# hidayetersindursun/LangSplatV2

Measured on AMD Instinct MI355X. Metric: frames/s fwd+bwd @ 1M Gaussians 1080p 3+16ch; achieved HBM GB/s, higher is better.
Workload: dtype f32; 1 GPU; BASELINE cfg3: 1M Gaussians, 1920x1080, SH deg 3 + 16 dense language channels, fwd+bwd, all inputs require grad; 1 view per GPU; gaussians=1000000, width=1920, height=1080, lang_dim=16, sh_degree=3, global_batch=1, parallelism=single GPU

## Files before the change

### langsplatv2_amd/csrc/binning.hip

```cpp
#include "bin_common.h"

#include <algorithm>

#ifndef LSR_BIN_TARGET
#define LSR_BIN_TARGET 512
#endif
#ifndef LSR_SORT_WAVE_MAX
#define LSR_SORT_WAVE_MAX 1024
#endif
#ifndef LSR_SORT_DPP
#define LSR_SORT_DPP 1
#endif

namespace lsr {

#define SCAN_ITEMS 16
#define SCAN_BLOCK 256
#define SCAN_TILE (SCAN_ITEMS * SCAN_BLOCK)

size_t scan_partials(size_t n) { return (n + SCAN_TILE - 1) / SCAN_TILE + 1; }

template <int NB>
__device__ __forceinline__ uint64_t block_excl_scan_u64_n(uint64_t v, uint64_t* sh, uint64_t& total)
{
    const int lane = threadIdx.x & 63, w = threadIdx.x >> 6;
    uint64_t x = v;
#pragma unroll
    for (int d = 1; d < 64; d <<= 1) {
        uint64_t y = __shfl_up(x, d, 64);
        if (lane >= d) x += y;
    }
    if (lane == 63) sh[w] = x;
    __syncthreads();
    uint64_t wofs = 0, tot = 0;
    for (int k = 0; k < NB / 64; k++) {
        if (k < w) wofs += sh[k];
        tot += sh[k];
    }
    __syncthreads();
    total = tot;
    return wofs + x - v;
}
__device__ __forceinline__ uint64_t block_excl_scan_u64(uint64_t v, uint64_t* sh, uint64_t& total)
{
    return block_excl_scan_u64_n<SCAN_BLOCK>(v, sh, total);
}

__global__ void __launch_bounds__(SCAN_BLOCK) k_scan_reduce(const uint32_t* __restrict__ in, size_t n,
                                                            uint64_t* __restrict__ part)
{
    __shared__ uint64_t sh[SCAN_BLOCK / 64];
    const size_t base = (size_t)blockIdx.x * SCAN_TILE + (size_t)threadIdx.x * SCAN_ITEMS;
    uint64_t s = 0;
#pragma unroll
    for (int k = 0; k < SCAN_ITEMS; k++)
        if (base + k < n) s += in[base + k];
    uint64_t tot;
    block_excl_scan_u64(s, sh, tot);
    if (threadIdx.x == 0) part[blockIdx.x] = tot;
}

__global__ void __launch_bounds__(SCAN_BLOCK) k_scan_part(uint64_t* __restrict__ part, int nb)
{
    __shared__ uint64_t sh[SCAN_BLOCK / 64];
    uint64_t carry = 0;
    for (int base = 0; base < nb; base += SCAN_BLOCK) {
        const int i = base + threadIdx.x;
        uint64_t v = i < nb ? part[i] : 0;
        uint64_t tot;
        uint64_t ex = block_excl_scan_u64(v, sh, tot);
        __syncthreads();
        if (i < nb) part[i] = carry + ex;
        carry += tot;
        __syncthreads();
    }
    if (threadIdx.x == 0) part[nb] = carry;
}

__global__ void __launch_bounds__(SCAN_BLOCK) k_scan_apply(const uint32_t* __restrict__ in, uint32_t* __restrict__ out,
                                                           size_t n, const uint64_t* __restrict__ part, int exclusive)
{
    __shared__ uint64_t sh[SCAN_BLOCK / 64];
    const size_t base = (size_t)blockIdx.x * SCAN_TILE + (size_t)threadIdx.x * SCAN_ITEMS;
    uint32_t v[SCAN_ITEMS];
    uint64_t s = 0;
#pragma unroll
    for (int k = 0; k < SCAN_ITEMS; k++) {
        v[k] = (base + k < n) ? in[base + k] : 0u;
        s += v[k];
    }
    uint64_t tot;
    uint64_t run = block_excl_scan_u64(s, sh, tot) + part[blockIdx.x];
#pragma unroll
    for (int k = 0; k < SCAN_ITEMS; k++) {
        const uint64_t incl = run + v[k];
        if (base + k < n) out[base + k] = (uint32_t)(exclusive ? run : incl);
        run = incl;
    }
}

hipError_t launch_scan_u32(const uint32_t* in, uint32_t* out, uint64_t* part, size_t n, bool exclusive, hipStream_t st)
{
    const int nb = (int)((n + SCAN_TILE - 1) / SCAN_TILE);
    if (nb > 0) k_scan_reduce<<<nb, SCAN_BLOCK, 0, st>>>(in, n, part);
    k_scan_part<<<1, SCAN_BLOCK, 0, st>>>(part, nb);
    if (nb > 0) k_scan_apply<<<nb, SCAN_BLOCK, 0, st>>>(in, out, n, part, exclusive ? 1 : 0);
    return hipGetLastError();
}

__global__ void k_publish_total(const uint64_t* __restrict__ total, uint32_t* __restrict__ tile_end,
                                uint64_t* host_slot, uint32_t seq, const uint32_t* __restrict__ cls_cnt)
{
    const uint64_t m = *total;
    const uint32_t m32 = m >= 0xffffffffull ? 0xffffffffu : (uint32_t)m;
    if (tile_end) *tile_end = m32;
    if (cls_cnt) {
        uint32_t* h = (uint32_t*)(host_slot + 1);
#pragma unroll
        for (int k = 0; k < SORT_NCLS; k++) h[k] = cls_cnt[k];
        __atomic_store_n(host_slot + LSR_CLS_SLOT, ((uint64_t)seq << 32) | m32, __ATOMIC_RELEASE);
    }
    __atomic_store_n(host_slot, ((uint64_t)seq << 32) | m32, __ATOMIC_RELEASE);
}

hipError_t launch_publish_total(const uint64_t* total, uint32_t* tile_end, uint64_t* host_slot, uint32_t seq,
                                const uint32_t* cls_cnt, hipStream_t st)
{
    k_publish_total<<<1, 1, 0, st>>>(total, tile_end, host_slot, seq, cls_cnt);
    return hipGetLastError();
}

__device__ __forceinline__ int tile_class(int n)
{
    if (n <= 0) return -1;
    if (n <= LSR_SORT_WAVE_MAX) return 0;
    if (n <= 1024) return 1;
    if (n <= 2048) return 2;
    if (n <= 4096) return 3;
    if (n <= 8192) return 4;
    return 5;
}

__device__ __forceinline__ void tile_class_append(bool active, int t, int n, int T, uint32_t* __restrict__ cls_cnt,
                                                  uint32_t* __restrict__ cls_list)
{
    const int c = active ? tile_class(n) : -1;
    const int lane = threadIdx.x & 63;
    const uint64_t below = lane ? (~0ull >> (64 - lane)) : 0ull;
    uint64_t m[SORT_NCLS];
    uint32_t cnt = 0;
#pragma unroll
    for (int k = 0; k < SORT_NCLS; k++) {
        m[k] = __ballot(c == k);
        cnt = lane == k ? (uint32_t)__popcll(m[k]) : cnt;
    }
    uint32_t base = 0;
    if (cnt) base = atomicAdd(&cls_cnt[lane], cnt);
    uint64_t mine = 0;
#pragma unroll
    for (int k = 0; k < SORT_NCLS; k++) mine = c == k ? m[k] : mine;
    const uint32_t b = __shfl(base, c < 0 ? 0 : c, 64);
    if (c >= 0) cls_list[(size_t)c * T + b + __popcll(mine & below)] = (uint32_t)t;
}

__global__ void __launch_bounds__(256) k_tile_classify(int T, const uint32_t* __restrict__ tile_start,
                                                       uint32_t* __restrict__ cls_cnt, uint32_t* __restrict__ cls_list)
{
    const int t = blockIdx.x * 256 + threadIdx.x;
    const int n = t < T ? (int)(tile_start[t + 1] - tile_start[t]) : 0;
    tile_class_append(t < T, t, n, T, cls_cnt, cls_list);
}

__global__ void __launch_bounds__(256) k_duplicate(Cam c, int P, const uint8_t* __restrict__ geom,
                                                   const int32_t* __restrict__ radii, uint32_t* __restrict__ tile_cnt,
                                                   uint32_t* __restrict__ rank)
{
    const int i = blockIdx.x * blockDim.x + threadIdx.x;
    if (i >= P) return;
    const int r = radii[i];
    if (r <= 0) return;
    const GeomLayout L = geom_layout(P);
    const float4 A = ((const float4*)(geom + L.splatA))[i];
    const float4 B = ((const float4*)(geom + L.splatB))[i];
    const uint32_t* tiles = (const uint32_t*)(geom + L.tiles);
    const uint32_t* offs = (const uint32_t*)(geom + L.offsets);
    uint32_t o = offs[i] - tiles[i];
    int x0, y0, x1, y1;
    get_rect(A.x, A.y, r, c.gx, c.gy, x0, y0, x1, y1);
    const SpanPrep sp = span_prep(A, B);
    int bx0 = x0, by0 = y0, bx1 = x1, by1 = y1;
    cull_box(A.x, A.y, A.z, A.w, B.x, B.z, bx0, by0, bx1, by1);
    for (int y = y0; y < y1; y++) {
        int sx0 = 0, sx1 = 0;
        if (y >= by0 && y < by1) row_span(sp, y, bx0, bx1, sx0, sx1);
        for (int x = x0; x < x1; x++, o++)
            rank[o] = (x >= sx0 && x < sx1) ? atomicAdd(&tile_cnt[y * c.gx + x], 1u) : 0xffffffffu;
    }
}

hipError_t launch_duplicate(const Cam& c, int P, const uint8_t* geom, const int32_t* radii, uint32_t* tile_cnt,
                            uint32_t* rank, hipStream_t st)
{
    if (P == 0) return hipSuccess;
    k_duplicate<<<(P + 255) / 256, 256, 0, st>>>(c, P, geom, radii, tile_cnt, rank);
    return hipGetLastError();
}

__global__ void __launch_bounds__(256) k_scatter(Cam c, int P, const uint8_t* __restrict__ geom,
                                                 const int32_t* __restrict__ radii,
                                                 const uint32_t* __restrict__ tile_start,
                                                 const uint32_t* __restrict__ rank, uint64_t* __restrict__ keys)
{
    const int i = blockIdx.x * blockDim.x + threadIdx.x;
    if (i >= P) return;
    const int r = radii[i];
    if (r <= 0) return;
    const GeomLayout L = geom_layout(P);
    const float4 A = ((const float4*)(geom + L.splatA))[i];
    const float depth = ((const float*)(geom + L.depth))[i];
    const uint32_t* tiles = (const uint32_t*)(geom + L.tiles);
    const uint32_t* offs = (const uint32_t*)(geom + L.offsets);
    uint32_t o = offs[i] - tiles[i];
    const uint64_t key = ((uint64_t)__float_as_uint(depth) << 32) | (uint32_t)i;
    int x0, y0, x1, y1;
    get_rect(A.x, A.y, r, c.gx, c.gy, x0, y0, x1, y1);
    for (int y = y0; y < y1; y++)
        for (int x = x0; x < x1; x++, o++)
            if (rank[o] != 0xffffffffu) keys[tile_start[y * c.gx + x] + rank[o]] = key;
}

hipError_t launch_scatter(const Cam& c, int P, const uint8_t* geom, const int32_t* radii, const uint32_t* tile_start,
                          const uint32_t* rank, uint64_t* keys, hipStream_t st)
{
    if (P == 0) return hipSuccess;
    k_scatter<<<(P + 255) / 256, 256, 0, st>>>(c, P, geom, radii, tile_start, rank, keys);
    return hipGetLastError();
}



struct WaveSpans {
    int rpre[65];
    int epre[65];
    float4 P0[64];
    float4 P1[64];
    float me[64];
    int box[64];
    int y0[64];
    int ent[64];
};

__device__ __forceinline__ int wave_spans_stage(WaveSpans& ws, int h, int bx0, int bx1, int y0, const SpanPrep& sp)
{
    const int lane = threadIdx.x & 63;
    ws.P0[lane] = make_float4(sp.x, sp.y, sp.vm, sp.vr);
    ws.P1[lane] = make_float4(sp.cb, sp.det, sp.tca, sp.ica);
    ws.me[lane] = sp.me;
    ws.box[lane] = bx0 | (bx1 << 16);
    ws.y0[lane] = y0;
    int s = h;
#pragma unroll
    for (int d = 1; d < 64; d <<= 1) {
        const int t = __shfl_up(s, d, 64);
        if (lane >= d) s += t;
    }
    ws.rpre[lane] = s - h;
    if (lane == 63) ws.rpre[64] = s;
    wave_lds_fence();
    return __shfl(s, 63, 64);
}

__device__ __forceinline__ int row_entry(const WaveSpans& ws, int e, int ty0, int& sx0, int& sx1, int& yr)
{
    const int o = wave_search(ws.rpre, e);
    yr = ws.y0[o] + (e - ws.rpre[o]);
    const float4 p0 = ws.P0[o], p1 = ws.P1[o];
    const SpanPrep sp{p0.x, p0.y, p0.z, p0.w, p1.x, p1.y, p1.z, p1.w, ws.me[o]};
    const int bx = ws.box[o];
    row_span(sp, yr + ty0, bx & 0xffff, bx >> 16, sx0, sx1);
    return o;
}

__device__ __forceinline__ int wave_spans_round(WaveSpans& ws, int r0, int R, int ty0)
{
    const int lane = threadIdx.x & 63;
    const int e = r0 + lane;
    int wd = 0, packed = 0;
    if (e < R) {
        int sx0, sx1, yr;
        const int o = row_entry(ws, e, ty0, sx0, sx1, yr);
        wd = sx1 - sx0;
        packed = sx0 | (yr << 16) | (o << 24);
    }
    int s = wd;
#pragma unroll
    for (int d = 1; d < 64; d <<= 1) {
        const int t = __shfl_up(s, d, 64);
        if (lane >= d) s += t;
    }
    ws.epre[lane] = s - wd;
    if (lane == 63) ws.epre[64] = s;
    ws.ent[lane] = packed;
    wave_lds_fence();
    return __shfl(s, 63, 64);
}

struct SpanWalk {
    int j, x, xe, y, o;
    __device__ __forceinline__ void enter(const WaveSpans& ws, int k0)
    {
        const int p = ws.ent[j];
        x = (p & 0xffff) + k0;
        xe = (p & 0xffff) + (ws.epre[j + 1] - ws.epre[j]);
        y = (p >> 16) & 0xff;
        o = p >> 24;
    }
    __device__ __forceinline__ SpanWalk(const WaveSpans& ws, int k)
    {
        j = wave_search(ws.epre, k);
        enter(ws, k - ws.epre[j]);
    }
    __device__ __forceinline__ void next(const WaveSpans& ws)
    {
        if (++x < xe) return;
        do { ++j; } while (ws.epre[j + 1] == ws.epre[j]);
        enter(ws, 0);
    }
};

__device__ __forceinline__ int stage_gaussian(WaveSpans& ws, const Cam& c, const Band& bd, const BinRec& g)
{
    int x0, x1, y0;
    const int h = band_box(c, bd, g, x0, x1, y0);
    return wave_spans_stage(ws, h, x0, x1, y0, span_prep(g.A, g.B));
}

template <int BB>
__global__ void __launch_bounds__(BB) k_bin_count(Cam c, int P, int chunk, int rows, int S,
                                                         const uint8_t* __restrict__ geom,
                                                         const int32_t* __restrict__ radii, uint32_t* __restrict__ table,
                                                         uint32_t* __restrict__ cls_cnt, uint64_t* host_slot, uint32_t seq)
{
    extern __shared__ uint32_t hist[];
    __shared__ WaveSpans wss[BB / 64];
    __shared__ uint64_t s_tot;
    const int T = c.gx * c.gy;
#if LSR_COUNT_XCD
    const int o = xcd_remap(blockIdx.x, gridDim.x);
    const int blk = o / S;
    const Band bd(c, rows, o - blk * S);
#else
    const int blk = blockIdx.x;
    const Band bd(c, rows, blockIdx.y);
#endif
    if (blockIdx.x == 0 && blockIdx.y == 0 && threadIdx.x < SORT_NCLS) cls_cnt[threadIdx.x] = 0;
    if (blockIdx.x == 0 && blockIdx.y == 0 && threadIdx.x == 0) cls_cnt[LSR_TICKET_WORD] = 0;
    for (int k = threadIdx.x; k < bd.nt; k += BB) hist[k] = 0;
    if (threadIdx.x == 0) s_tot = 0;
    __syncthreads();
    WaveSpans& ws = wss[threadIdx.x >> 6];
    const int lane = threadIdx.x & 63;
    const int g0 = blk * chunk, g1 = min(P, g0 + chunk);
    BinRec nx;
    if (g0 < g1) nx.load(geom, P, g1, radii, g0 + (threadIdx.x & ~63) + lane, false);
    for (int i0 = g0 + (threadIdx.x & ~63); i0 < g1; i0 += BB) {
        const BinRec cur = nx;
        nx.load(geom, P, g1, radii, i0 + BB + lane, false);
        const int R = stage_gaussian(ws, c, bd, cur);
        for (int e = lane; e < R; e += 64) {
            int sx0, sx1, yr;
            row_entry(ws, e, bd.ty0, sx0, sx1, yr);
            if (sx1 > sx0) {
                atomicAdd(&hist[yr * c.gx + sx0], 1u);
                if (sx1 < c.gx) atomicAdd(&hist[yr * c.gx + sx1], 0xffffffffu);
            }
        }
        wave_lds_fence();
    }
    __syncthreads();
    uint32_t* row = table + (size_t)blk * table_stride(T) + bd.t0;
    const int nrows = bd.ty1 - bd.ty0;
    uint64_t mine = 0;
    for (int r = threadIdx.x >> 6; r < nrows; r += BB / 64) {
        uint32_t carry = 0;
        for (int x0 = 0; x0 < c.gx; x0 += 64) {
            const int x = x0 + lane;
            uint32_t v = x < c.gx ? hist[r * c.gx + x] : 0u;
#pragma unroll
            for (int d = 1; d < 64; d <<= 1) {
                const uint32_t t = __shfl_up(v, d, 64);
                if (lane >= d) v += t;
            }
            if (x < c.gx) {
                row[r * c.gx + x] = carry + v;
                mine += carry + v;
            }
            carry += __shfl(v, 63, 64);
        }
    }
#pragma unroll
    for (int d = 32; d >= 1; d >>= 1) mine += __shfl_xor(mine, d, 64);
    if (lane == 0 && mine) atomicAdd((unsigned long long*)&s_tot, (unsigned long long)mine);
    __syncthreads();
    if (threadIdx.x == 0) {
        const uint64_t add = s_tot + (1ull << 44);
        const uint64_t prev = __hip_atomic_fetch_add((uint64_t*)(cls_cnt + LSR_COUNT_WORD), add, __ATOMIC_RELAXED,
                                                     __HIP_MEMORY_SCOPE_AGENT);
        if ((prev >> 44) == (uint64_t)gridDim.x * gridDim.y - 1) {
            const uint64_t m = (prev + add) & ((1ull << 44) - 1);
            const uint32_t m32 = m >= 0xffffffffull ? 0xffffffffu : (uint32_t)m;
            __hip_atomic_store(host_slot, ((uint64_t)seq << 32) | m32, __ATOMIC_RELAXED, __HIP_MEMORY_SCOPE_SYSTEM);
        }
    }
}

#define TBL_TILES 64
#define TBL_RPT 16
struct BinPublish {
    uint64_t* gpart;
    uint32_t* ticket;
    uint32_t* tile_end;
    uint64_t* host_slot;
    uint32_t seq;
};
__device__ __forceinline__ uint32_t u4_get(const uint4& v, int j) { return j == 0 ? v.x : j == 1 ? v.y : j == 2 ? v.z : v.w; }
__device__ __forceinline__ uint4 u4_add(const uint4& a, const uint4& b)
{
    return make_uint4(a.x + b.x, a.y + b.y, a.z + b.z, a.w + b.w);
}

template <int SEGS>
__global__ void __launch_bounds__(16 * SEGS) k_bin_table(int T, int Tp, int B, uint32_t* __restrict__ table,
                                                         uint32_t* __restrict__ tile_cnt,
                                                         uint32_t* __restrict__ cls_cnt,
                                                         uint32_t* __restrict__ cls_list, BinPublish pb)
{
    constexpr int NT = 16 * SEGS;
    __shared__ uint4 seg_sum[SEGS][16];
    __shared__ uint64_t sh[NT / 64];
    __shared__ int s_last;
    const int cg = threadIdx.x & 15, seg = threadIdx.x >> 4;
    const int t4 = blockIdx.x * TBL_TILES + cg * 4;
    const int b0 = seg * TBL_RPT;
    const uint4 cmask = make_uint4(t4 < T ? ~0u : 0u, t4 + 1 < T ? ~0u : 0u, t4 + 2 < T ? ~0u : 0u,
                                   t4 + 3 < T ? ~0u : 0u);
    const bool colok = t4 < Tp;
    uint4 v[TBL_RPT];
    uint4 sum = make_uint4(0u, 0u, 0u, 0u);
#pragma unroll
    for (int k = 0; k < TBL_RPT; k++) {
        const int b = b0 + k;
        uint4 x = make_uint4(0u, 0u, 0u, 0u);
        if (colok && b < B) x = *reinterpret_cast<const uint4*>(table + (size_t)b * Tp + t4);
        v[k] = make_uint4(x.x & cmask.x, x.y & cmask.y, x.z & cmask.z, x.w & cmask.w);
        sum = u4_add(sum, v[k]);
    }
    seg_sum[seg][cg] = sum;
    __syncthreads();
    uint4 run = make_uint4(0u, 0u, 0u, 0u), tot = run;
    for (int k = 0; k < SEGS; k++) {
        const uint4 x = seg_sum[k][cg];
        if (k < seg) run = u4_add(run, x);
        tot = u4_add(tot, x);
    }
    if (threadIdx.x < 64) {
        const int l = threadIdx.x, src = l >> 2, j = l & 3;
        const uint32_t n0 = __shfl(tot.x, src, 64), n1 = __shfl(tot.y, src, 64);
        const uint32_t n2 = __shfl(tot.z, src, 64), n3 = __shfl(tot.w, src, 64);
        const uint32_t nl = j == 0 ? n0 : j == 1 ? n1 : j == 2 ? n2 : n3;
        const int tl = blockIdx.x * TBL_TILES + l;
        tile_class_append(tl < T, tl, (int)nl, T, cls_cnt, cls_list);
        uint64_t g = seg == 0 ? (uint64_t)tot.x + tot.y + tot.z + tot.w : 0ull;
#pragma unroll
        for (int d = 8; d >= 1; d >>= 1) g += __shfl_xor(g, d, 64);
        if (threadIdx.x == 0) __hip_atomic_store(&pb.gpart[blockIdx.x], g, __ATOMIC_RELAXED, __HIP_MEMORY_SCOPE_AGENT);
        if (seg == 0) {
#pragma unroll
            for (int j = 0; j < 4; j++)
                if (t4 + j < T) tile_cnt[t4 + j] = u4_get(tot, j);
        }
    }
    if (colok) {
#pragma unroll
        for (int k = 0; k < TBL_RPT; k++) {
            const int b = b0 + k;
            if (b < B) *reinterpret_cast<uint4*>(table + (size_t)b * Tp + t4) = run;
            run = u4_add(run, v[k]);
        }
    }
    asm volatile("s_waitcnt vmcnt(0)" ::: "memory");
    __syncthreads();
    if (threadIdx.x == 0) {
        const uint32_t prev = __hip_atomic_fetch_add(pb.ticket, 1u, __ATOMIC_RELAXED, __HIP_MEMORY_SCOPE_AGENT);
        s_last = prev == gridDim.x - 1;
    }
    __syncthreads();
    if (!s_last) return;
    __builtin_amdgcn_fence(__ATOMIC_ACQUIRE, "wavefront");
    const int G = (int)gridDim.x;
    uint64_t carry = 0;
    for (int base = 0; base < G; base += NT * 8) {
        const int i0 = base + threadIdx.x * 8;
        uint64_t gv[8], s = 0;
#pragma unroll
        for (int k = 0; k < 8; k++)
            gv[k] = i0 + k < G ? __hip_atomic_load(&pb.gpart[i0 + k], __ATOMIC_RELAXED, __HIP_MEMORY_SCOPE_AGENT) : 0ull;
#pragma unroll
        for (int k = 0; k < 8; k++) s += gv[k];
        uint64_t gt;
        uint64_t r = carry + block_excl_scan_u64_n<NT>(s, sh, gt);
#pragma unroll
        for (int k = 0; k < 8; k++) {
            if (i0 + k < G) pb.gpart[i0 + k] = r;
            r += gv[k];
        }
        carry += gt;
    }
    if (threadIdx.x < 64) {
        const int l = threadIdx.x;
        const uint32_t cnt = l < SORT_NCLS ? __hip_atomic_load(&cls_cnt[l], __ATOMIC_RELAXED, __HIP_MEMORY_SCOPE_AGENT) : 0u;
        uint32_t cv[SORT_NCLS];
#pragma unroll
        for (int k = 0; k < SORT_NCLS; k++) cv[k] = __shfl(cnt, k, 64);
        if (l == 0) {
            const uint32_t m32 = carry >= 0xffffffffull ? 0xffffffffu : (uint32_t)carry;
            pb.gpart[G] = carry;
            *pb.tile_end = m32;
            uint32_t* h = (uint32_t*)(pb.host_slot - LSR_CLS_SLOT + 1);
#pragma unroll
            for (int k = 0; k < SORT_NCLS; k++) __hip_atomic_store(&h[k], cv[k], __ATOMIC_RELAXED, __HIP_MEMORY_SCOPE_SYSTEM);
            asm volatile("s_waitcnt vmcnt(0)" ::: "memory");
            __hip_atomic_store(pb.host_slot, ((uint64_t)pb.seq << 32) | m32, __ATOMIC_RELAXED, __HIP_MEMORY_SCOPE_SYSTEM);
        }
    }
}

__global__ void __launch_bounds__(256) k_tile_start_apply(int T, const uint32_t* __restrict__ tile_cnt,
                                                          const uint64_t* __restrict__ gpart,
                                                          uint32_t* __restrict__ tile_start)
{
    const int t = blockIdx.x * 256 + threadIdx.x;
    const uint32_t v = t < T ? tile_cnt[t] : 0u;
    uint32_t x = v;
    const int l = threadIdx.x & 63;
#pragma unroll
    for (int d = 1; d < 64; d <<= 1) {
        const uint32_t y = __shfl_up(x, d, 64);
        if (l >= d) x += y;
    }
    if (t < T) tile_start[t] = (uint32_t)gpart[t / TBL_TILES] + x - v;
}

template <int BB>
__global__ void __launch_bounds__(BB) k_bin_scatter(Cam c, int P, int chunk, int km, int rows, int S,
                                                           const uint8_t* __restrict__ geom,
                                                           const int32_t* __restrict__ radii,
                                                           const uint32_t* __restrict__ table,
                                                           const uint32_t* __restrict__ tile_start,
                                                           uint64_t* __restrict__ keys)
{
    extern __shared__ uint32_t base[];
    __shared__ WaveSpans wss[BB / 64];
    __shared__ uint64_t wkey[BB];
    const int T = c.gx * c.gy;
    const int o = xcd_remap(blockIdx.x, gridDim.x);
    const int blk = (o / S) * km;
    const Band bd(c, rows, o - (o / S) * S);
    const uint32_t* row = table + (size_t)blk * table_stride(T) + bd.t0;
    for (int k = threadIdx.x; k < bd.nt; k += BB) base[k] = tile_start[bd.t0 + k] + row[k];
    __syncthreads();
    WaveSpans& ws = wss[threadIdx.x >> 6];
    uint64_t* const key = wkey + (threadIdx.x & ~63);
    const int lane = threadIdx.x & 63;
    const int g0 = blk * chunk, g1 = min(P, g0 + km * chunk);
    BinRec nx;
    if (g0 < g1) nx.load(geom, P, g1, radii, g0 + (threadIdx.x & ~63) + lane, true);
    for (int i0 = g0 + (threadIdx.x & ~63); i0 < g1; i0 += BB) {
        const int i = i0 + lane;
        const BinRec cur = nx;
        nx.load(geom, P, g1, radii, i0 + BB + lane, true);
        key[lane] = ((uint64_t)__float_as_uint(cur.depth) << 32) | (uint32_t)i;
        const int R = stage_gaussian(ws, c, bd, cur);
        for (int r0 = 0; r0 < R; r0 += 64) {
            const int K = wave_spans_round(ws, r0, R, bd.ty0);
            const int q = (K + 63) >> 6;
            int k = lane * q;
            const int kend = min(K, k + q);
            if (k < kend) {
                SpanWalk sw(ws, k);
                for (;;) {
                    const uint32_t sa = atomicAdd(&base[sw.y * c.gx + sw.x], 1u);
                    const uint64_t ka = key[sw.o];
                    const bool two = k + 1 < kend;
                    uint32_t sb = 0;
                    uint64_t kb = 0;
                    if (two) {
                        sw.next(ws);
                        sb = atomicAdd(&base[sw.y * c.gx + sw.x], 1u);
                        kb = key[sw.o];
                    }
                    keys[sa] = ka;
                    if (two) keys[sb] = kb;
                    k += 2;
                    if (k >= kend) break;
                    sw.next(ws);
                }
            }
            wave_lds_fence();
        }
    }
}

#ifndef LSR_BAND_ROWS
#define LSR_BAND_ROWS 34
#endif
#ifndef LSR_BAND_ROWS_SMALL
#define LSR_BAND_ROWS_SMALL 68
#endif
static int bin_band_rows(const Cam& c, int P)
{
    const bool big = P >= (4 << 20);
    const int cap = big ? LSR_BAND_ROWS : LSR_BAND_ROWS_SMALL;
    const int lds = big ? LSR_BAND_LDS : 2 * LSR_BAND_LDS;
    return std::max(1, std::min(std::min(c.gy, cap), lds / (4 * c.gx)));
}

#ifndef LSR_SCATTER_LDS
#define LSR_SCATTER_LDS LSR_BAND_LDS
#endif
#ifndef LSR_SCATTER_ROWS
#define LSR_SCATTER_ROWS 0
#endif
#ifndef LSR_SCATTER_MERGE
#define LSR_SCATTER_MERGE 0
#endif
int scatter_merge(int P) { return LSR_SCATTER_MERGE > 0 ? LSR_SCATTER_MERGE : (P >= (4 << 20) ? 4 : 1); }
int bin_scatter_rows(const Cam& c)
{
    if (LSR_SCATTER_ROWS > 0) return std::max(1, std::min(c.gy, LSR_SCATTER_ROWS));
    return std::max(1, std::min(c.gy, LSR_SCATTER_LDS / (4 * c.gx)));
}

int bin_block(int P) { return P >= (4 << 20) ? 512 : 1024; }

int bin_blocks(int P, const Cam& c, int& chunk)
{
    const int rows = bin_band_rows(c, P);
    const int S = (c.gy + rows - 1) / rows;
    const int total = P >= (4 << 20) ? 2 * LSR_BIN_TARGET : LSR_BIN_TARGET;
    const int target = std::max(64, total / S);
    chunk = max(1024, (P + target - 1) / target);
    const int bb = bin_block(P);
    chunk = (chunk + bb - 1) / bb * bb;
    return (P + chunk - 1) / chunk;
}

bool bin_privatised_ok(const Cam& c) { return (size_t)c.gx * 4 <= LSR_BAND_LDS && (size_t)c.gx * c.gy <= (1u << 20); }

hipError_t launch_bin_count(const Cam& c, int P, int chunk, int B, const uint8_t* geom, const int32_t* radii,
                            uint32_t* table, uint32_t* tile_cnt, uint32_t* tile_start, uint64_t* tpart,
                            uint32_t* cls_cnt, uint32_t* cls_list, uint64_t* host_slot, uint32_t seq, hipStream_t st)
{
    const int T = c.gx * c.gy;
    const int rows = bin_band_rows(c, P);
    const int S = (c.gy + rows - 1) / rows;
    const dim3 grid(LSR_COUNT_XCD ? B * S : B, LSR_COUNT_XCD ? 1 : S);
    const size_t lds = (size_t)rows * c.gx * 4;
    if (lds > 65536) {
        (void)hipFuncSetAttribute((const void*)k_bin_count<512>, hipFuncAttributeMaxDynamicSharedMemorySize, (int)lds);
        (void)hipFuncSetAttribute((const void*)k_bin_scatter<512>, hipFuncAttributeMaxDynamicSharedMemorySize, (int)lds);
        (void)hipFuncSetAttribute((const void*)k_bin_scatter<1024>, hipFuncAttributeMaxDynamicSharedMemorySize, (int)lds);
    }
    if (B > 0) {
        if ((size_t)grid.x * grid.y >= (1u << 20)) return hipErrorInvalidValue;
        k_bin_count<512><<<grid, 512, lds, st>>>(c, P, chunk, rows, S, geom, radii, table, cls_cnt, host_slot, seq);
        BinPublish pb{tpart, cls_cnt + LSR_TICKET_WORD, tile_start + T, host_slot + LSR_CLS_SLOT, seq};
        const int G = (T + TBL_TILES - 1) / TBL_TILES, Tp = table_stride(T);
        if (B <= 16 * TBL_RPT)
            k_bin_table<16><<<G, 256, 0, st>>>(T, Tp, B, table, tile_cnt, cls_cnt, cls_list, pb);
        else if (B <= 32 * TBL_RPT)
            k_bin_table<32><<<G, 512, 0, st>>>(T, Tp, B, table, tile_cnt, cls_cnt, cls_list, pb);
        else if (B <= 64 * TBL_RPT)
            k_bin_table<64><<<G, 1024, 0, st>>>(T, Tp, B, table, tile_cnt, cls_cnt, cls_list, pb);
        else
            return hipErrorInvalidValue;
    } else {
        (void)hipMemsetAsync(tile_cnt, 0, (size_t)T * 4, st);
        (void)hipMemsetAsync(cls_cnt, 0, SORT_NCLS * 4, st);
        (void)launch_scan_u32(tile_cnt, tile_start, tpart, (size_t)T, true, st);
        (void)launch_publish_total(tpart + (scan_partials((size_t)T) - 1), tile_start + T, host_slot, seq, cls_cnt, st);
    }
    return hipGetLastError();
}

hipError_t launch_tile_start_apply(int T, int B, const uint32_t* tile_cnt, const uint64_t* tpart, uint32_t* tile_start,
                                   hipStream_t st)
{
    if (B > 0 && T > 0) k_tile_start_apply<<<(T + 255) / 256, 256, 0, st>>>(T, tile_cnt, tpart, tile_start);
    return hipGetLastError();
}

hipError_t launch_bin_scatter(const Cam& c, int P, int chunk, int B, const uint8_t* geom, const int32_t* radii,
                              const uint32_t* table, const uint32_t* tile_start, uint64_t* keys, hipStream_t st)
{
    const int rows = bin_scatter_rows(c);
    const int S = (c.gy + rows - 1) / rows;
    const size_t lds = (size_t)rows * c.gx * 4;
    if (lds > 65536) {
        (void)hipFuncSetAttribute((const void*)k_bin_scatter<512>, hipFuncAttributeMaxDynamicSharedMemorySize, (int)lds);
        (void)hipFuncSetAttribute((const void*)k_bin_scatter<1024>, hipFuncAttributeMaxDynamicSharedMemorySize, (int)lds);
    }
    const int km = scatter_merge(P), Bs = (B + km - 1) / km;
    if (B > 0 && bin_block(P) == 1024)
        k_bin_scatter<1024><<<Bs * S, 1024, lds, st>>>(c, P, chunk, km, rows, S, geom, radii, table, tile_start, keys);
    else if (B > 0)
        k_bin_scatter<512><<<Bs * S, 512, lds, st>>>(c, P, chunk, km, rows, S, geom, radii, table, tile_start, keys);
    return hipGetLastError();
}

#define SORT_BLOCK 256
#define SORT_CHUNK 4096

__device__ __forceinline__ void ce(uint64_t* a, int i, int l)
{
    uint64_t x = a[i], y = a[l];
    if (x > y) { a[i] = y; a[l] = x; }
}

__device__ void bitonic_lds(uint64_t* a, int n, int kmax)
{
    for (int k = 2; k <= kmax; k <<= 1) {
        const int hk = k >> 1;
        for (int p = threadIdx.x; p < kmax / 2; p += SORT_BLOCK) {
            const int blk = p / hk, off = p % hk;
            const int i = blk * k + off, l = blk * k + k - 1 - off;
            if (l < n) ce(a, i, l);
        }
        __syncthreads();
        for (int j = k >> 2; j >= 1; j >>= 1) {
            for (int p = threadIdx.x; p < kmax / 2; p += SORT_BLOCK) {
                const int i = (p / j) * 2 * j + (p % j), l = i + j;
                if (l < n) ce(a, i, l);
            }
            __syncthreads();
        }
    }
}

__device__ void halfclean_lds(uint64_t* a, int n, int chunk, int jmax)
{
    for (int j = jmax; j >= 1; j >>= 1) {
        for (int p = threadIdx.x; p < chunk / 2; p += SORT_BLOCK) {
            const int i = (p / j) * 2 * j + (p % j), l = i + j;
            if (l < n) ce(a, i, l);
        }
        __syncthreads();
    }
}

__device__ __forceinline__ int next_pow2(int n)
{
    int p = 1;
    while (p < n) p <<= 1;
    return p;
}

__device__ void tile_sort_big(int t, const uint32_t* __restrict__ tile_start, uint64_t* __restrict__ keys,
                              uint32_t* __restrict__ point_list, uint64_t* buf)
{
    const uint32_t s0 = tile_start[t], s1 = tile_start[t + 1];
    const int n = (int)(s1 - s0);
    uint64_t* g = keys + s0;
    if (n <= SORT_CHUNK) {
        for (int k = threadIdx.x; k < n; k += SORT_BLOCK) buf[k] = g[k];
        __syncthreads();
        bitonic_lds(buf, n, next_pow2(n));
        for (int k = threadIdx.x; k < n; k += SORT_BLOCK) point_list[s0 + k] = (uint32_t)buf[k];
        __syncthreads();
        return;
    }
    const int n2 = next_pow2(n);
    const int nch = (n + SORT_CHUNK - 1) / SORT_CHUNK;
    for (int ch = 0; ch < nch; ch++) {
        const int cb = ch * SORT_CHUNK, cn = min(SORT_CHUNK, n - cb);
        for (int k = threadIdx.x; k < cn; k += SORT_BLOCK) buf[k] = g[cb + k];
        __syncthreads();
        bitonic_lds(buf, cn, SORT_CHUNK);
        for (int k = threadIdx.x; k < cn; k += SORT_BLOCK) g[cb + k] = buf[k];
        __syncthreads();
    }
    for (int k = 2 * SORT_CHUNK; k <= n2; k <<= 1) {
        const int hk = k >> 1;
        for (int p = threadIdx.x; p < n2 / 2; p += SORT_BLOCK) {
            const int blk = p / hk, off = p % hk;
            const int i = blk * k + off, l = blk * k + k - 1 - off;
            if (l < n) ce(g, i, l);
        }
        __syncthreads();
        for (int j = k >> 2; j >= SORT_CHUNK; j >>= 1) {
            for (int p = threadIdx.x; p < n2 / 2; p += SORT_BLOCK) {
                const int i = (p / j) * 2 * j + (p % j), l = i + j;
                if (l < n) ce(g, i, l);
            }
            __syncthreads();
        }
        for (int ch = 0; ch < nch; ch++) {
            const int cb = ch * SORT_CHUNK, cn = min(SORT_CHUNK, n - cb);
            for (int q = threadIdx.x; q < cn; q += SORT_BLOCK) buf[q] = g[cb + q];
            __syncthreads();
            halfclean_lds(buf, cn, SORT_CHUNK, SORT_CHUNK / 2);
            for (int q = threadIdx.x; q < cn; q += SORT_BLOCK) g[cb + q] = buf[q];
            __syncthreads();
        }
    }
    for (int k = threadIdx.x; k < n; k += SORT_BLOCK) point_list[s0 + k] = (uint32_t)g[k];
    __syncthreads();
}

__global__ void __launch_bounds__(SORT_BLOCK) k_tile_sort_big(int T, const uint32_t* __restrict__ tile_start,
                                                              uint64_t* __restrict__ keys,
                                                              uint32_t* __restrict__ point_list,
                                                              const uint32_t* __restrict__ cls_cnt,
                                                              const uint32_t* __restrict__ cls_list)
{
    __shared__ uint64_t buf[SORT_CHUNK];
    const uint32_t cnt = cls_cnt[5];
    for (uint32_t i = blockIdx.x; i < cnt; i += gridDim.x)
        tile_sort_big((int)cls_list[(size_t)5 * T + i], tile_start, keys, point_list, buf);
}

__device__ __forceinline__ uint64_t shfl_xor_u64(uint64_t v, int m)
{
    const uint32_t lo = __shfl_xor((uint32_t)v, m, 64);
    const uint32_t hi = __shfl_xor((uint32_t)(v >> 32), m, 64);
    return ((uint64_t)hi << 32) | lo;
}

#ifndef LSR_SORT_XBATCH
#define LSR_SORT_XBATCH 1
#endif
template <int M>
__device__ __forceinline__ uint64_t xor_lane_u64(uint64_t v)
{
#if LSR_SORT_DPP
    const uint32_t lo = xor_lane_u32<M>((uint32_t)v);
    const uint32_t hi = xor_lane_u32<M>((uint32_t)(v >> 32));
    return ((uint64_t)hi << 32) | lo;
#else
    return shfl_xor_u64(v, M);
#endif
}

template <int KPL, int K, int J>
__device__ __forceinline__ void wave_sort_xstep(uint64_t (&v)[KPL])
{
    constexpr int M = J / KPL;
    const int lane = threadIdx.x & 63;
    const bool take_min = ((lane & M) == 0) == (((lane * KPL) & K) == 0);
#if LSR_SORT_XBATCH
    uint64_t o[KPL];
#pragma unroll
    for (int r = 0; r < KPL; r++) o[r] = xor_lane_u64<M>(v[r]);
#pragma unroll
    for (int r = 0; r < KPL; r++) v[r] = ((v[r] < o[r]) == take_min) ? v[r] : o[r];
#else
#pragma unroll
    for (int r = 0; r < KPL; r++) {
        const uint64_t o = xor_lane_u64<M>(v[r]);
        v[r] = ((v[r] < o) == take_min) ? v[r] : o;
    }
#endif
}

template <int KPL, int K, int J>
__device__ __forceinline__ void wave_sort_steps(uint64_t (&v)[KPL])
{
    if constexpr (J >= 1) {
        if constexpr (J < KPL) {
            const int lane = threadIdx.x & 63;
            const bool desc_lane = ((lane * KPL) & K) != 0;
#pragma unroll
            for (int r = 0; r < KPL; r++) {
                if (r & J) continue;
                const uint64_t a = v[r], b = v[r | J];
                bool sw;
                if constexpr (K < KPL) sw = (r & K) ? (a < b) : (a > b);
                else sw = (a > b) != desc_lane;
                v[r] = sw ? b : a;
                v[r | J] = sw ? a : b;
            }
        } else {
            wave_sort_xstep<KPL, K, J>(v);
        }
        wave_sort_steps<KPL, K, J / 2>(v);
    }
}

template <int KPL, int K>
__device__ __forceinline__ void wave_sort_stages(uint64_t (&v)[KPL])
{
    if constexpr (K <= 64 * KPL) {
        wave_sort_steps<KPL, K, K / 2>(v);
        wave_sort_stages<KPL, 2 * K>(v);
    }
}

template <int KPL>
__device__ __forceinline__ void wave_sort_tile(const uint64_t* __restrict__ g, uint32_t* __restrict__ out, int n)
{
    const int lane = threadIdx.x & 63;
    uint64_t v[KPL];
#pragma unroll
    for (int r = 0; r < KPL; r++) {
        const int e = lane * KPL + r;
        v[r] = e < n ? g[e] : ~0ull;
    }
    wave_sort_stages<KPL, 2>(v);
#pragma unroll
    for (int r = 0; r < KPL; r++) {
        const int e = lane * KPL + r;
        if (e < n) out[e] = (uint32_t)v[r];
    }
}

__device__ __forceinline__ int lpad(int e) { return e + (e >> 4); }

__device__ __forceinline__ int merge_corank(const uint64_t* lds, int a0, int na, int b0, int nb, int d)
{
    int lo = max(0, d - nb), hi = min(d, na);
    while (lo < hi) {
        const int m = (lo + hi) >> 1;
        if (lds[lpad(a0 + m)] < lds[lpad(b0 + d - 1 - m)]) lo = m + 1;
        else hi = m;
    }
    return lo;
}

template <int KPL>
__device__ __forceinline__ void merge_run(const uint64_t* lds, int a0, int na, int b0, int nb, int d,
                                          uint64_t (&v)[KPL])
{
    int i = merge_corank(lds, a0, na, b0, nb, d), j = d - i;
    uint64_t a = i < na ? lds[lpad(a0 + i)] : ~0ull, b = j < nb ? lds[lpad(b0 + j)] : ~0ull;
#pragma unroll
    for (int k = 0; k < KPL; k++) {
        const bool ta = a < b;
        v[k] = ta ? a : b;
        i += ta ? 1 : 0;
        j += ta ? 0 : 1;
        const bool ok = ta ? (i < na) : (j < nb);
        const uint64_t nx = ok ? lds[lpad(ta ? a0 + i : b0 + j)] : ~0ull;
        a = ta ? nx : a;
        b = ta ? b : nx;
    }
}

template <int KPL>
__device__ __forceinline__ void block_sort_tile(const uint64_t* __restrict__ g, uint32_t* __restrict__ out, int n,
                                                uint64_t* lds)
{
    constexpr int R = 64 * KPL;
    const int tid = threadIdx.x, lane = tid & 63, w = tid >> 6;
#pragma unroll 1
    for (int k0 = 0; k0 < 4 * KPL; k0 += 8) {
        uint64_t x[8];
#pragma unroll
        for (int k = 0; k < 8; k++) {
            const int e = (k0 + k) * 256 + tid;
            x[k] = e < n ? g[e] : ~0ull;
        }
#pragma unroll
        for (int k = 0; k < 8; k++) lds[lpad((k0 + k) * 256 + tid)] = x[k];
    }
    __syncthreads();
    uint64_t v[KPL];
#pragma unroll
    for (int r = 0; r < KPL; r++) v[r] = lds[lpad(w * R + lane * KPL + r)];
    wave_sort_stages<KPL, 2>(v);
#pragma unroll
    for (int r = 0; r < KPL; r++) lds[lpad(w * R + lane * KPL + r)] = v[r];
    __syncthreads();
    {
        const int p0 = (tid >> 7) * 2 * R, d = (tid & 127) * KPL;
        merge_run<KPL>(lds, p0, R, p0 + R, R, d, v);
        __syncthreads();
#pragma unroll
        for (int k = 0; k < KPL; k++) lds[lpad(p0 + d + k)] = v[k];
    }
    __syncthreads();
    const int d = tid * KPL;
    merge_run<KPL>(lds, 0, 2 * R, 2 * R, 2 * R, d, v);
    __syncthreads();
    uint32_t* l32 = (uint32_t*)lds;
#pragma unroll
    for (int k = 0; k < KPL; k++) l32[d + k + ((d + k) >> 5)] = (uint32_t)v[k];
    __syncthreads();
#pragma unroll 8
    for (int e = tid; e < n; e += 256) out[e] = l32[e + (e >> 5)];
    __syncthreads();
}

template <int KPL>
__global__ void __launch_bounds__(256) k_tile_sort_blk(int T, const uint32_t* __restrict__ tile_start,
                                                       const uint64_t* __restrict__ keys,
                                                       uint32_t* __restrict__ point_list,
                                                       const uint32_t* __restrict__ cls_cnt,
                                                       const uint32_t* __restrict__ cls_list, int cls)
{
    __shared__ uint64_t lds[(4 * 64 * KPL) * 17 / 16];
    const uint32_t cnt = cls_cnt[cls];
    for (uint32_t i = blockIdx.x; i < cnt; i += gridDim.x) {
        const int t = (int)cls_list[(size_t)cls * T + i];
        const uint32_t s0 = tile_start[t];
        block_sort_tile<KPL>(keys + s0, point_list + s0, (int)(tile_start[t + 1] - s0), lds);
    }
}

__global__ void __launch_bounds__(256) k_tile_sort_wave(int T, const uint32_t* __restrict__ tile_start,
                                                        const uint64_t* __restrict__ keys,
                                                        uint32_t* __restrict__ point_list,
                                                        const uint32_t* __restrict__ cls_cnt,
                                                        const uint32_t* __restrict__ cls_list)
{
    const uint32_t cnt = cls_cnt[0];
    for (uint32_t i = blockIdx.x * 4 + (threadIdx.x >> 6); i < cnt; i += gridDim.x * 4) {
        const int t = (int)cls_list[i];
        const uint32_t s0 = tile_start[t];
        const int n = (int)(tile_start[t + 1] - s0);
        const uint64_t* g = keys + s0;
        uint32_t* o = point_list + s0;
        if (n == 1) {
            if ((threadIdx.x & 63) == 0) o[0] = (uint32_t)g[0];
        } else if (n <= 64) wave_sort_tile<1>(g, o, n);
        else if (n <= 128) wave_sort_tile<2>(g, o, n);
        else if (n <= 256) wave_sort_tile<4>(g, o, n);
        else if (LSR_SORT_WAVE_MAX <= 512 || n <= 512) wave_sort_tile<8>(g, o, n);
        else if (LSR_SORT_WAVE_MAX <= 1024 || n <= 1024) wave_sort_tile<16>(g, o, n);
        else wave_sort_tile<32>(g, o, n);
    }
}

hipError_t launch_tile_sort(int T, const uint32_t* tile_start, uint64_t* keys, uint32_t* point_list,
                            uint32_t* cls_cnt, uint32_t* cls_list, const uint32_t* host_cnt, hipStream_t st)
{
    if (T == 0) return hipSuccess;
    uint32_t cnt[SORT_NCLS];
    if (host_cnt) {
        for (int k = 0; k < SORT_NCLS; k++) cnt[k] = host_cnt[k];
    } else {
        (void)hipMemsetAsync(cls_cnt, 0, SORT_NCLS * 4, st);
        k_tile_classify<<<(T + 255) / 256, 256, 0, st>>>(T, tile_start, cls_cnt, cls_list);
        const uint32_t fill[SORT_NCLS] = {256 * 8, 256 * 8, 256 * 8, 256 * 4, 256 * 2, 256 * 2};
        for (int k = 0; k < SORT_NCLS; k++) cnt[k] = std::min<uint32_t>((uint32_t)T, fill[k] * (k == 0 ? 4 : 1));
    }
    const uint32_t* cc = cls_cnt;
    const uint32_t* cl = cls_list;
    if (cnt[0]) k_tile_sort_wave<<<(cnt[0] + 3) / 4, 256, 0, st>>>(T, tile_start, keys, point_list, cc, cl);
    if (cnt[1]) k_tile_sort_blk<4><<<cnt[1], 256, 0, st>>>(T, tile_start, keys, point_list, cc, cl, 1);
    if (cnt[2]) k_tile_sort_blk<8><<<cnt[2], 256, 0, st>>>(T, tile_start, keys, point_list, cc, cl, 2);
    if (cnt[3]) k_tile_sort_blk<16><<<cnt[3], 256, 0, st>>>(T, tile_start, keys, point_list, cc, cl, 3);
    if (cnt[4]) k_tile_sort_blk<32><<<cnt[4], 256, 0, st>>>(T, tile_start, keys, point_list, cc, cl, 4);
    if (cnt[5]) k_tile_sort_big<<<cnt[5], SORT_BLOCK, 0, st>>>(T, tile_start, keys, point_list, cc, cl);
    return hipGetLastError();
}

}
```

Before: 947.0 frames/s.

## Replace wave bitonic sort with in-register lane sort plus cross-lane merge

Each lane now sorts its keys in registers first, then runs cross-lane merge stages that use flipped xor exchanges and half-cleaners. KPL may now be any even value (plus 3), so tiles are padded much less than with power-of-two sizes. The goal is fewer cross-lane shuffles and less wasted compare work on padding keys. The kernel also gets a waves-per-EU hint, and a static_assert caps the wave sort at 16 keys per lane, which adds template instantiations and code size.

```diff
diff --git a/langsplatv2_amd/csrc/binning.hip b/langsplatv2_amd/csrc/binning.hip
--- a/langsplatv2_amd/csrc/binning.hip
+++ b/langsplatv2_amd/csrc/binning.hip
@@ -8,6 +8,7 @@
 #ifndef LSR_SORT_WAVE_MAX
 #define LSR_SORT_WAVE_MAX 1024
 #endif
+static_assert(LSR_SORT_WAVE_MAX == 512 || LSR_SORT_WAVE_MAX == 1024, "the one-wave sort holds at most 16 keys per lane");
 #ifndef LSR_SORT_DPP
 #define LSR_SORT_DPP 1
 #endif
@@ -906,6 +907,61 @@
 }
 
 template <int KPL>
+__device__ __forceinline__ void lane_sort_regs(uint64_t (&v)[KPL])
+{
+#pragma unroll
+    for (int p = 1; p < KPL; p *= 2) {
+#pragma unroll
+        for (int k = p; k >= 1; k /= 2) {
+#pragma unroll
+            for (int j = k % p; j + k < KPL; j += 2 * k) {
+#pragma unroll
+                for (int i = 0; i < k; i++) {
+                    const int a = i + j, b = i + j + k;
+                    if (b >= KPL || a / (2 * p) != b / (2 * p)) continue;
+                    const uint64_t x = v[a], y = v[b];
+                    const bool sw = x > y;
+                    v[a] = sw ? y : x;
+                    v[b] = sw ? x : y;
+                }
+            }
+        }
+    }
+}
+
+template <int KPL, int M, int LOW, bool FLIP>
+__device__ __forceinline__ void wsort_xstep(uint64_t (&v)[KPL])
+{
+    const int lane = threadIdx.x & 63;
+    const bool take_min = (lane & LOW) == 0;
+    uint64_t o[KPL];
+#pragma unroll
+    for (int r = 0; r < KPL; r++) o[r] = xor_lane_u64<M>(v[FLIP ? KPL - 1 - r : r]);
+#pragma unroll
+    for (int r = 0; r < KPL; r++) v[r] = ((v[r] < o[r]) == take_min) ? v[r] : o[r];
+}
+
+template <int KPL, int D>
+__device__ __forceinline__ void wsort_halfclean(uint64_t (&v)[KPL])
+{
+    if constexpr (D >= 1) {
+        wsort_xstep<KPL, D, D, false>(v);
+        wsort_halfclean<KPL, D / 2>(v);
+    }
+}
+
+template <int KPL, int M>
+__device__ __forceinline__ void wsort_merge_lanes(uint64_t (&v)[KPL])
+{
+    if constexpr (M <= 64) {
+        wsort_xstep<KPL, M - 1, M / 2, true>(v);
+        wsort_halfclean<KPL, M / 4>(v);
+        lane_sort_regs<KPL>(v);
+        wsort_merge_lanes<KPL, 2 * M>(v);
+    }
+}
+
+template <int KPL>
 __device__ __forceinline__ void wave_sort_tile(const uint64_t* __restrict__ g, uint32_t* __restrict__ out, int n)
 {
     const int lane = threadIdx.x & 63;
@@ -915,7 +971,8 @@
         const int e = lane * KPL + r;
         v[r] = e < n ? g[e] : ~0ull;
     }
-    wave_sort_stages<KPL, 2>(v);
+    lane_sort_regs<KPL>(v);
+    wsort_merge_lanes<KPL, 2>(v);
 #pragma unroll
     for (int r = 0; r < KPL; r++) {
         const int e = lane * KPL + r;
@@ -1016,7 +1073,8 @@
     }
 }
 
-__global__ void __launch_bounds__(256) k_tile_sort_wave(int T, const uint32_t* __restrict__ tile_start,
+__global__ void __launch_bounds__(256) __attribute__((amdgpu_waves_per_eu(4)))
+k_tile_sort_wave(int T, const uint32_t* __restrict__ tile_start,
                                                         const uint64_t* __restrict__ keys,
                                                         uint32_t* __restrict__ point_list,
                                                         const uint32_t* __restrict__ cls_cnt,
@@ -1031,12 +1089,22 @@
         uint32_t* o = point_list + s0;
         if (n == 1) {
             if ((threadIdx.x & 63) == 0) o[0] = (uint32_t)g[0];
-        } else if (n <= 64) wave_sort_tile<1>(g, o, n);
-        else if (n <= 128) wave_sort_tile<2>(g, o, n);
-        else if (n <= 256) wave_sort_tile<4>(g, o, n);
-        else if (LSR_SORT_WAVE_MAX <= 512 || n <= 512) wave_sort_tile<8>(g, o, n);
-        else if (LSR_SORT_WAVE_MAX <= 1024 || n <= 1024) wave_sort_tile<16>(g, o, n);
-        else wave_sort_tile<32>(g, o, n);
+            continue;
+        }
+        int kpl = (n + 63) >> 6;
+        if (kpl > 4) kpl = (kpl + 1) & ~1;
+        switch (kpl) {
+        case 1: wave_sort_tile<1>(g, o, n); break;
+        case 2: wave_sort_tile<2>(g, o, n); break;
+        case 3: wave_sort_tile<3>(g, o, n); break;
+        case 4: wave_sort_tile<4>(g, o, n); break;
+        case 6: wave_sort_tile<6>(g, o, n); break;
+        case 8: wave_sort_tile<8>(g, o, n); break;
+        case 10: wave_sort_tile<10>(g, o, n); break;
+        case 12: wave_sort_tile<12>(g, o, n); break;
+        case 14: wave_sort_tile<14>(g, o, n); break;
+        default: wave_sort_tile<16>(g, o, n); break;
+        }
     }
 }
 
```

Result: faster. 956.4 frames/s (median of 6 runs) (+1.0%).
